# victorvde/jpeg2png

Hardware: NVIDIA H100
Metric: Mpixel-iterations/s (higher is better)
Workload: dtype f32

## Files before the change

jpeg2png_b200/csrc/kernels_project.cu:

```cuda
#include <cuda_runtime.h>
#include <stdint.h>
#include <stdlib.h>

#include "kernels.cuh"
#include "project_generic_body.cuh"
#include "numerics.cuh"
#include "project_common.cuh"
#include "strip_sync.cuh"
#include "tma_maps.h"


namespace j2p {

cudaError_t launch_project_tile(const FrameDev &F, int c, int count, float factor, cudaStream_t s, int *nlaunch, bool uncovered_only);
cudaError_t configure_project_tma();
bool project_tma_enabled();
cudaError_t launch_project_tma(const FrameDev &F, const TileMaps &M, int c, int count, int xsel, float factor, cudaStream_t s);
cudaError_t configure_project_tile22();
cudaError_t launch_project_tile22(const FrameDev &F, int c, int count, float factor, cudaStream_t s, int *nlaunch, bool uncovered_only);

template <int SW, int SH>
__global__ void __launch_bounds__(P_NT, (SW * SH <= 1) ? J2P_PROJ_MIN_CTAS : 2) k_project(const __grid_constant__ FrameDev F, const ProjPlane G, const float factor) {
    constexpr bool REC = false;
    const RecDev R{};
#include "project_generic_body.inc"
}

struct QTable { float q[64]; };
__global__ void __launch_bounds__(P_NT) k_decode(const int16_t *data, const __grid_constant__ QTable qt, float *out, int cw, int ch) {
    const float *q = qt.q;
    __shared__ __align__(16) float tiles[P_NT / 8][TILE_STRIDE];
    const int tid = threadIdx.x, b = tid >> 3, j = tid & 7;
    const int nb = (cw >> 3) * (ch >> 3);
    const int blk = blockIdx.x * (P_NT / 8) + b;
    if (blk >= nb) return;
    const int bw = cw >> 3, by = blk / bw, bx = blk - by * bw;
    float v[8];
// ... 24 lines not shown

cudaError_t configure_project_kernels() {
    const char *e = getenv("J2P_PROJ_TILE22");
    g_tile22 = !(e && *e == '0');
    const cudaError_t rc = configure_project_tma();
    return rc != cudaSuccess ? rc : configure_project_tile22();
}

__global__ void k_fold_sums(const double *sums_by_rank, int nranks, int nc, float *norms) {
    const int c = threadIdx.x;
    if (c >= nc) return;
    double s = 0.;
    for (int r = 0; r < nranks; r++) s = __dadd_rn(s, sums_by_rank[r * 3 + c]);
    const float norm = fsqrt(__double2float_rn(s));
    norms[c] = norm;
    norms[4 + c] = __frcp_rn(norm);
}

cudaError_t launch_fold_sums(const double *sums_by_rank, int nranks, int nc, float *norms, cudaStream_t s) {
    k_fold_sums<<<1, 32, 0, s>>>(sums_by_rank, nranks, nc, norms);
    return cudaGetLastError();
}

cudaError_t launch_project(const FrameDev &Fin, float factor, cudaStream_t s, int *nlaunch) {
    *nlaunch = 0;
    FrameDev F = Fin;
    if (F.t0 != 0 || F.t1 != F.H) {
        const size_t off = (size_t)F.t0 * F.W;
        for (int c = 0; c < F.nc; c++) {
            F.pl[c].x += off;
            F.pl[c].xp += off;
            F.pl[c].g += off;
        }
        F.H = F.t1 - F.t0;
    }
    for (int c = 0; c < F.nc; c++) {
        const PlaneDev &P = F.pl[c];
        const int tw = 8 * P_BW * P.sw, th = 8 * P_BH * P.sh;
        ProjPlane G;
        G.c = c;
        G.gx = (F.W + tw - 1) / tw;
        const int gy = (F.H + th - 1) / th;
        auto each_rows = [&](const FrameDev &V, auto launch) {
            for (int y0 = 0; y0 < gy; y0 += kMaxGridRows) {
                const int rows = gy - y0 < kMaxGridRows ? gy - y0 : kMaxGridRows;
                launch(y0 == 0 && rows == gy ? V : rows_view(V, c, 1, y0 * P_BH, 8 * P.sh, y0 + rows == gy), dim3(G.gx, rows));
                *nlaunch += 1;
            }
        };
        if (F.log_on && P.sw == 1 && P.sh == 1) {
            each_rows(F, [&](const FrameDev &V, dim3 grid) { k_project<1, 1><<<grid, P_NT, 0, s>>>(V, G, factor); });
        } else if (P.sw == 1 && P.sh == 1) {
            int count = 1;
            while (c + count < F.nc && F.pl[c + count].sw == 1 && F.pl[c + count].sh == 1 && F.pl[c + count].cw == P.cw &&
                   F.pl[c + count].ch == P.ch)
                count++;
            const bool tma = Fin.host_maps != nullptr && project_tma_enabled();
            if (tma) {
                const cudaError_t et = launch_project_tma(Fin, *static_cast<const TileMaps *>(Fin.host_maps), c, count, Fin.buf_sel, factor, s);
                if (et != cudaSuccess) return et;
                *nlaunch += 1;
            }
            const cudaError_t eb = launch_project_tile(F, c, count, factor, s, nlaunch, tma);
            if (eb != cudaSuccess) return eb;
            c += count - 1;
        }
        else if (P.sw == 2 && P.sh == 2 && g_tile22 && !F.log_on) {
            int count = 1;
            while (c + count < F.nc && F.pl[c + count].sw == 2 && F.pl[c + count].sh == 2 && F.pl[c + count].cw == P.cw &&
                   F.pl[c + count].ch == P.ch)
                count++;
            const cudaError_t eb = launch_project_tile22(F, c, count, factor, s, nlaunch, false);
            if (eb != cudaSuccess) return eb;
            c += count - 1;
        }
        else {
            for (int f = 0; f < F.nframes; f++) {
                each_rows(F.nframes > 1 ? frame_view(F, f) : F, [&](const FrameDev &V, dim3 grid) {
                    if (P.sw == 2 && P.sh == 2) k_project<2, 2><<<grid, P_NT, 0, s>>>(V, G, factor);
                    else if (P.sw == 2 && P.sh == 1) k_project<2, 1><<<grid, P_NT, 0, s>>>(V, G, factor);
                    else if (P.sw == 1 && P.sh == 2) k_project<1, 2><<<grid, P_NT, 0, s>>>(V, G, factor);
                    else k_project<0, 0><<<grid, P_NT, 0, s>>>(V, G, factor);
                });
            }
        }
        const cudaError_t e = cudaGetLastError();
// ... 24 lines not shown
```

jpeg2png_b200/csrc/kernels_project_tile.cu:

```cuda
#include <cuda_runtime.h>
#include <stdint.h>

#include "project_tile_body.cuh"

namespace j2p {

template <bool RES, bool BATCH>
__global__ void __launch_bounds__(PT_NT, J2P_TILE_MIN_CTAS) k_project_tile(const __grid_constant__ FrameDev F, const int c0, const float factor) {
    const GridGeo geo{};
    constexpr bool REC = false;
    const RecDev R{};
#include "project_tile_body.inc"
}

template <bool BATCH>
__global__ void k_step_uncovered(const __grid_constant__ FrameDev F, const int c, const float factor) {
    step_uncovered_body<BATCH>(F, c, factor, GridGeo{});
}

static cudaError_t launch_step_uncovered(const FrameDev &F, int c, float factor, cudaStream_t s) {
    const PlaneDev &P = F.pl[c];
    const size_t n = (size_t)(F.H - P.ch) * F.W + (size_t)P.ch * (F.W - P.cw);
    int blocks = (int)((n + 255) / 256);
    if (F.nframes > 1) {
        const int cap = (132 * 8 + F.nframes - 1) / F.nframes;
        k_step_uncovered<true><<<dim3(blocks < cap ? blocks : cap, 1, F.nframes), 256, 0, s>>>(F, c, factor);
        return cudaGetLastError();
    }
    if (blocks > 132 * 8) blocks = 132 * 8;
    k_step_uncovered<false><<<blocks, 256, 0, s>>>(F, c, factor);
    return cudaGetLastError();
}

int project_tile_border_units(const PlaneDev &P) { return ((P.cw >> 3) + PT_NB - 1) / PT_NB; }

cudaError_t launch_project_tile(const FrameDev &F, int c, int count, float factor, cudaStream_t s, int *nlaunch, bool uncovered_only) {
    const PlaneDev &P = F.pl[c];
    const int bw = P.cw >> 3, bh = P.ch >> 3, gx = (bw + PT_NB - 1) / PT_NB;
    const bool batch = F.nframes > 1;
    cudaError_t e = cudaSuccess;
    for (int y0 = 0; y0 < bh && !uncovered_only && e == cudaSuccess; y0 += kMaxGridRows) {
        const int rows = bh - y0 < kMaxGridRows ? bh - y0 : kMaxGridRows;
        const FrameDev V = y0 == 0 && rows == bh ? F : rows_view(F, c, count, y0, 8, y0 + rows == bh);
        const dim3 grid = batch ? dim3(gx * count, rows, F.nframes) : dim3(gx, rows, count);
        if (batch)
            e = P.resample ? launch_chain(k_project_tile<true, true>, grid, dim3(PT_NT), 0, s, V, c, factor) : launch_chain(k_project_tile<false, true>, grid, dim3(PT_NT), 0, s, V, c, factor);
        else
            e = P.resample ? launch_chain(k_project_tile<true, false>, grid, dim3(PT_NT), 0, s, V, c, factor) : launch_chain(k_project_tile<false, false>, grid, dim3(PT_NT), 0, s, V, c, factor);
        *nlaunch += 1;
    }
    for (int k = c; k < c + count && e == cudaSuccess; k++)
        if (F.pl[k].cw < F.W || F.pl[k].ch < F.H) {
            e = launch_step_uncovered(F, k, factor, s);
            *nlaunch += 1;
        }
    return e;
}

}
```

jpeg2png_b200/csrc/pdl.cuh:

```cuda
#pragma once
#include <cuda_runtime.h>
#include <stdlib.h>

#include <utility>

namespace j2p {

#ifdef __CUDACC__
__device__ __forceinline__ void pdl_wait() { asm volatile("griddepcontrol.wait;" ::: "memory"); }
__device__ __forceinline__ void pdl_launch_dependents() { asm volatile("griddepcontrol.launch_dependents;" ::: "memory"); }
#endif

inline bool pdl_enabled() {
    static const bool on = [] {
        const char *e = getenv("J2P_PDL");
        return !(e && *e == '0');
    }();
    return on;
}

template <typename... KArgs, typename... Args>
inline cudaError_t launch_chain(void (*kernel)(KArgs...), dim3 grid, dim3 block, size_t smem, cudaStream_t s, Args &&...args) {
    cudaLaunchConfig_t cfg = {};
    cfg.gridDim = grid;
    cfg.blockDim = block;
    cfg.dynamicSmemBytes = smem;
    cfg.stream = s;
    cudaLaunchAttribute attr[1];
    attr[0].id = cudaLaunchAttributeProgrammaticStreamSerialization;
    attr[0].val.programmaticStreamSerializationAllowed = pdl_enabled() ? 1 : 0;
    cfg.attrs = attr;
    cfg.numAttrs = 1;
    return cudaLaunchKernelEx(&cfg, kernel, std::forward<Args>(args)...);
}

}
```

jpeg2png_b200/csrc/session.cu:

```cuda
#include <cuda_runtime.h>

#include <math.h>
#include <stdarg.h>
#include <stdio.h>
#include <stdlib.h>
#include <string.h>
#include <sys/mman.h>
#include <time.h>

#include <atomic>
#include <algorithm>
#include <map>
#include <string>
#include <mutex>
#include <utility>
#include <vector>

#include "../../include/jpeg2png_b200.h"
#include "copy_pool.h"
#include "geometry.cuh"
#include "kernels.cuh"
#include "record.cuh"
#include "tma_maps.h"

namespace j2p {
int grad_cta_count(int W, int H);
cudaError_t configure_kernels(int *slots);
cudaError_t launch_gradient(const FrameDev &F, float factor, cudaStream_t s);
cudaError_t launch_project(const FrameDev &F, float factor, cudaStream_t s, int *nlaunch);
cudaError_t launch_fold_sums(const double *sums_by_rank, int nranks, int nc, float *norms, cudaStream_t s);
cudaError_t launch_decode(const int16_t *data, const float *q_host, float *out, int cw, int ch, cudaStream_t s);
cudaError_t launch_init_plane(const float *fdata, float *x, float *xp, int W, int H, int cw, int ch, int sw, int sh,
                              cudaStream_t s);
bool project_tma_enabled();
int project_tma_border_units(const PlaneDev &P);
int project_tile_border_units(const PlaneDev &P);
cudaError_t launch_scanlines(const EpilogueArgs &a, int nframes, cudaStream_t s, int *nlaunch);
cudaError_t launch_halo_exchange(const HaloPeers &P, unsigned seq, unsigned *ticket, int *err, int wait_for_arrival, cudaStream_t s);
int packed_gradient_gpm(const FrameDev &F);
void packed_gradient_geometry(const FrameDev &F, int *cx, int *bands, int *rows);
cudaError_t launch_project_tile(const FrameDev &F, int c, int count, float factor, cudaStream_t s, int *nlaunch, bool uncovered_only);
cudaError_t launch_project_tile22(const FrameDev &F, int c, int count, float factor, cudaStream_t s, int *nlaunch, bool uncovered_only);
}

using namespace j2p;

static thread_local char g_err[512] = "";

static int fail(int code, const char *fmt, ...) {
    va_list ap;
    va_start(ap, fmt);
    vsnprintf(g_err, sizeof g_err, fmt, ap);
    va_end(ap);
    return code;
}

#define CK(call)                                                                                      \
    do {                                                                                              \
        cudaError_t e_ = (call);                                                                      \
        if (e_ != cudaSuccess) {                                                                      \
            cudaGetLastError();    \
            return fail(J2P_ERR_CUDA, "%s failed: %s (%s:%d)", #call, cudaGetErrorString(e_), __FILE__, __LINE__); \
        }                                                                                             \
    } while (0)

constexpr int kEventRing = 32;
constexpr unsigned kEventStride = 4;

// ... 101 lines not shown
    unsigned next_iter = 0;
    unsigned long long launches = 0;
    int logging = 0;
    double log_host[8] = {};
    long long log_host_iter = -1;
    unsigned long long next_log_iter = 0;
    cudaEvent_t ev[kEventRing] = {};
    long long ev_iter[kEventRing];
    std::vector<std::pair<void *, size_t>> dev_blocks;
    void *stage[kStageSlots] = {};
    cudaEvent_t stage_ev[kStageSlots] = {};
    unsigned stage_next = 0;
    cudaEvent_t export_ev = nullptr;
    cudaEvent_t upload_ev = nullptr;
    unsigned long long uid = 0;
    unsigned long long tables_gen = 0;
    struct GroupPlan *group = nullptr;
    cudaEvent_t group_ev = nullptr;
    bool recording = false;
    bool rec_armed = false;
    double *rec_hist = nullptr;
    double *rec_pp = nullptr;
    unsigned rec_pp_stride = 0, rec_pp_count[3] = {};
};
static void free_group_plan(GroupPlan *g);

static void swap_iterates(FrameDev &F) {
    for (int c = 0; c < F.nc; c++) {
        PlaneDev &P = F.pl[c];
        float *tp = P.x; P.x = P.xp; P.xp = tp;
    }
    F.buf_sel ^= 1;
}

template <typename T>
static cudaError_t dev_alloc(j2p_session *s, T **p, size_t bytes) {
    bytes = bytes ? (bytes + 255) & ~(size_t)255 : 256;
    size_t got = bytes;
    void *q = g_dev_cache.get(s->device, bytes, &got);
    if (!q) {
        got = bytes;
        cudaError_t e = cudaMalloc(&q, bytes);
        if (e == cudaErrorMemoryAllocation) {
            cudaGetLastError();
            g_dev_cache.trim(s->device);
            e = cudaMalloc(&q, bytes);
// ... 51 lines not shown
    if (s && !x) fail(J2P_ERR_ARG, "plane %u out of range (%zu planes)", plane, s->uploaded.size());
    return x;
}
extern "C" unsigned long long j2p_session_launches(const j2p_session *s) { return s ? s->launches : 0; }

extern "C" void j2p_session_destroy(j2p_session *s) {
    if (!s) return;
    cudaSetDevice(s->device);
    if (s->stream) cudaStreamSynchronize(s->stream);
    for (auto &blk : s->dev_blocks)
        if (s->ipc_exported || !g_dev_cache.put(s->device, blk.first, blk.second)) cudaFree(blk.first);
    for (int i = 0; i < kEventRing; i++)
        if (s->ev[i]) cudaEventDestroy(s->ev[i]);
    for (int k = 0; k < kStageSlots; k++) {
        if (s->stage_ev[k]) cudaEventDestroy(s->stage_ev[k]);
        if (s->stage[k]) g_pinned.put(s->stage[k]);
    }
    if (s->export_ev) cudaEventDestroy(s->export_ev);
    if (s->upload_ev) cudaEventDestroy(s->upload_ev);
    if (s->group_ev) cudaEventDestroy(s->group_ev);
    free_group_plan(s->group);
    if (s->stream) cudaStreamDestroy(s->stream);
    delete s;
}

static int create_impl(j2p_session *s, int device, const j2p_frame_desc *d, unsigned row0, unsigned rows, unsigned nframes) {
    const int ndev = j2p_device_count();
    if (ndev <= 0) return fail(J2P_ERR_NODEVICE, "no CUDA device available (the solver has no CPU fallback)");
    if (device < 0 || device >= ndev) return fail(J2P_ERR_ARG, "device %d out of range (0..%d)", device, ndev - 1);
    if (d->nchannel < 1 || d->nchannel > 3) return fail(J2P_ERR_ARG, "nchannel must be 1..3 (compute.c:118)");
    s->device = device;
    s->desc = *d;
    CK(cudaSetDevice(device));
    if (device >= 64) return fail(J2P_ERR_ARG, "device ordinal %d not supported", device);
    std::call_once(g_cfg_once[device], [&] {
        int major = 0, minor = 0;
        cudaError_t e = cudaDeviceGetAttribute(&major, cudaDevAttrComputeCapabilityMajor, device);
        if (e == cudaSuccess) e = cudaDeviceGetAttribute(&minor, cudaDevAttrComputeCapabilityMinor, device);
        g_cfg_cc[device] = major * 10 + minor;
        g_cfg_err[device] = e != cudaSuccess ? e : (major * 10 + minor == 90 ? configure_kernels(&g_cfg_slots[device]) : cudaSuccess);
    });
    if (g_cfg_cc[device] != 90)
        return fail(J2P_ERR_NODEVICE, "device %d is sm_%d; this library is built for sm_90a only", device, g_cfg_cc[device]);
    CK(g_cfg_err[device]);

    FrameDev &F = s->F;
// ... 106 lines not shown
    for (unsigned c = 0; c < d->nchannel && maps_ok; c++) {
        const bool p11 = d->w_samp[c] == 1 && d->h_samp[c] == 1, p22 = d->w_samp[c] == 2 && d->h_samp[c] == 2;
        if (!p11 && !p22) continue;
        const int box_rows = p11 ? 8 : 16;
        maps_ok = encode_plane_map(&s->maps.m[c][0], s->x[c], F.W, F.H, box_rows) == 0 &&
                  encode_plane_map(&s->maps.m[c][1], s->xp[c], F.W, F.H, box_rows) == 0 &&
                  encode_plane_map(&s->maps.m[c][2], s->g[c], F.W, F.H, box_rows) == 0;
        if (maps_ok && p11) maps_ok = encode_plane_map(&s->maps.m[c][3], s->gp[c], F.pl[c].cw, F.pl[c].ch, 8) == 0;
    }
    F.host_maps = maps_ok ? &s->maps : nullptr;
    F.buf_sel = 0;
    F.grad_ctas = grad_cta_count(F.W, F.t1 - F.t0);
    F.grad_slots = g_cfg_slots[device];
    CK(dev_alloc(s, &F.partials, sizeof(double) * 5 * (size_t)F.grad_ctas * nframes));
    CK(dev_alloc(s, &F.norms, sizeof(float) * 16 * nframes));
    CK(dev_alloc(s, &F.sums, sizeof(double) * 4 * nframes));
    CK(dev_alloc(s, &F.logsums, sizeof(double) * 8));
    CK(cudaMemsetAsync(F.logsums, 0, sizeof(double) * 8, s->stream));
    F.log_on = 0;
    F.log_slot = 0;
    CK(dev_alloc(s, &F.counter, sizeof(unsigned) * nframes));
    CK(cudaMemsetAsync(F.counter, 0, sizeof(unsigned) * nframes, s->stream));
    CK(cudaMemsetAsync(F.norms, 0, sizeof(float) * 16 * nframes, s->stream));
    return J2P_OK;
}

extern "C" int j2p_session_create(j2p_session **out, int device, const struct j2p_frame_desc *d) {
    return j2p_session_create_strip(out, device, d, 0, 0);
}

static int create_session(j2p_session **out, int device, const struct j2p_frame_desc *d, unsigned row0, unsigned rows,
                          unsigned nframes) {
    if (!out || !d) return fail(J2P_ERR_ARG, "null argument");
    *out = nullptr;
    j2p_session *s = new j2p_session();
    static std::atomic<unsigned long long> uid_seq{0};
    s->uid = ++uid_seq;
    const int rc = create_impl(s, device, d, row0, rows, nframes);
    if (rc != J2P_OK) {
        char keep[sizeof g_err];
        memcpy(keep, g_err, sizeof keep);
        j2p_session_destroy(s);
        cudaGetLastError();
        memcpy(g_err, keep, sizeof keep);
        return rc;
    }
// ... 8 lines not shown

extern "C" int j2p_session_create_batch(j2p_session **out, int device, const struct j2p_frame_desc *d, unsigned nframes) {
    if (out) *out = nullptr;
    if (nframes == 0) return fail(J2P_ERR_ARG, "a batch needs at least one frame");
    if (nframes > 65535) return fail(J2P_ERR_ARG, "a batch holds at most 65535 frames (%u requested)", nframes);
    return create_session(out, device, d, 0, 0, nframes);
}

extern "C" unsigned j2p_session_frames(const j2p_session *s) { return s ? s->nframes : 0; }

static int refuse_batch(const j2p_session *s, const char *what) {
    return fail(J2P_ERR_ARG, "%s is not available on a batch session (%u frames)", what, s->nframes);
}

static int reset_impl(j2p_session *s) {
    FrameDev &F = s->F;
    for (size_t k = 0; k < s->uploaded.size(); k++)
        if (!s->uploaded[k]) return fail(J2P_ERR_ARG, "plane %zu (frame %zu, channel %zu) has not been uploaded", k, k / F.nc, k % F.nc);
    F.buf_sel = 0;
    for (int c = 0; c < F.nc; c++) {
        PlaneDev &P = F.pl[c];
        P.x = s->x[c];
        P.xp = s->xp[c];
    }
    for (unsigned f = 0; f < s->nframes; f++) {
        const size_t fo = (size_t)f * F.frame_stride;
        for (int c = 0; c < F.nc; c++) {
            PlaneDev &P = F.pl[c];
            const size_t off = (size_t)F.t0 * F.W;
            CK(launch_init_plane(s->fdata0[c] + f * s->fdata_stride, P.x + fo + off, P.xp + fo + off, F.W, F.t1 - F.t0, P.cw, P.ch, P.sw,
                                 P.sh, s->stream));
            s->launches++;
            CK(cudaMemsetAsync(P.gp + fo, 0, (size_t)P.cw * P.ch * sizeof(float), s->stream));
        }
    }
    if (s->dev_tables && s->tables_stale) {
        CK(cudaMemcpyAsync(s->dev_tables, s->tables.data(), s->tables.size() * sizeof(float), cudaMemcpyHostToDevice, s->stream));
        s->tables_stale = false;
    }
    s->stale = false;
    s->t = 1.f;
    s->next_iter = 0;
    for (int i = 0; i < kEventRing; i++) s->ev_iter[i] = -1;
    s->next_log_iter = 0;
    s->log_host_iter = -1;
    CK(cudaMemsetAsync(F.logsums, 0, sizeof(double) * 8, s->stream));
// ... 304 lines not shown
    if (!s) return fail(J2P_ERR_ARG, "null session");
    if (s->nframes > 1) return refuse_batch(s, "j2p_session_copy_halo_to_prev");
    CK(cudaSetDevice(s->device));
    const FrameDev &F = s->F;
    const size_t W = (size_t)F.W;
    for (int c = 0; c < F.nc; c++) {
        if (F.t0 > 0) CK(cudaMemcpyAsync(F.pl[c].xp, F.pl[c].x, (size_t)F.t0 * W * sizeof(float), cudaMemcpyDeviceToDevice, s->stream));
        if (F.t1 < F.H)
            CK(cudaMemcpyAsync(F.pl[c].xp + (size_t)F.t1 * W, F.pl[c].x + (size_t)F.t1 * W, (size_t)(F.H - F.t1) * W * sizeof(float),
                               cudaMemcpyDeviceToDevice, s->stream));
    }
    return J2P_OK;
}

extern "C" int j2p_session_strip_info(const j2p_session *s, unsigned *local_rows, unsigned *first_owned, unsigned *owned_rows) {
    if (!s) return fail(J2P_ERR_ARG, "null session");
    if (s->nframes > 1) return refuse_batch(s, "j2p_session_strip_info");
    if (local_rows) *local_rows = (unsigned)s->F.H;
    if (first_owned) *first_owned = (unsigned)s->F.t0;
    if (owned_rows) *owned_rows = (unsigned)(s->F.t1 - s->F.t0);
    return J2P_OK;
}

extern "C" int j2p_session_iterate(j2p_session *s, unsigned first, unsigned n) {
    if (!s) return fail(J2P_ERR_ARG, "null session");
    if (s->strip) return fail(J2P_ERR_ARG, "a strip session is driven with j2p_session_gradient / j2p_session_project");
    CK(cudaSetDevice(s->device));
    if (s->recording) {
        if ((unsigned long long)first + n > s->desc.iterations)
            return fail(J2P_ERR_ARG, "the objective record holds %u iterations; iterations %u..%llu asked for", s->desc.iterations, first,
                        (unsigned long long)first + n - 1);
        if (first != 0 && !s->rec_armed && !s->stale)
            return fail(J2P_ERR_ARG, "recording was switched on after iteration 0: iterate from first == 0 to re-arm the record");
    }
    int rc = check_ready(s, first);
    if (rc != J2P_OK) return rc;
    for (unsigned i = first; i < first + n; i++) {
        rc = one_iteration(s, i, nullptr, nullptr, nullptr);
        if (rc != J2P_OK) return rc;
        if (i % kEventStride == kEventStride - 1) {
            const int slot = (int)((i / kEventStride) % kEventRing);
            CK(cudaEventRecord(s->ev[slot], s->stream));
            s->ev_iter[slot] = (long long)i;
        }
    }
    s->next_iter = first + n;
    return J2P_OK;
}

extern "C" int j2p_session_profile(j2p_session *s, unsigned n, float *ms_gradient, float *ms_project) {
    if (!s || !ms_gradient || !ms_project || n == 0) return fail(J2P_ERR_ARG, "bad argument");
    CK(cudaSetDevice(s->device));
    if (s->recording && n > s->desc.iterations)
        return fail(J2P_ERR_ARG, "the objective record holds %u iterations; %u asked for", s->desc.iterations, n);
    int rc = check_ready(s, 0);
    if (rc != J2P_OK) return rc;
    cudaEvent_t e[3];
    for (int k = 0; k < 3; k++) CK(cudaEventCreate(&e[k]));
    double sg = 0., sp = 0.;
    for (unsigned i = 0; i < n; i++) {
        rc = one_iteration(s, i, e[0], e[1], e[2]);
        if (rc != J2P_OK) return rc;
        CK(cudaEventSynchronize(e[2]));
        float a = 0.f, b = 0.f;
        CK(cudaEventElapsedTime(&a, e[0], e[1]));
        CK(cudaEventElapsedTime(&b, e[1], e[2]));
// ... 345 lines not shown
    const FrameDev V = record_view(s);
    const RecDev R = record_args(s, iter);
    int cx, bands, rows;
    packed_gradient_geometry(V, &cx, &bands, &rows);
    CK((cudaError_t)objective_api().gradient(&V, factor, cx, bands, rows, packed_gradient_gpm(V), &R, (void *)s->stream));
    return J2P_OK;
}

static int record_project(j2p_session *s, unsigned iter, float factor, int *nlaunch) {
    const FrameDev V = record_view(s);
    const RecDev R = record_args(s, iter);
    *nlaunch = 0;
    for (int c = 0; c < V.nc; c++) {
        const PlaneDev &P = V.pl[c];
        const bool p11 = P.sw == 1 && P.sh == 1, p22 = P.sw == 2 && P.sh == 2;
        int count = 1;
        while ((p11 || p22) && c + count < V.nc && V.pl[c + count].sw == P.sw && V.pl[c + count].sh == P.sh && V.pl[c + count].cw == P.cw &&
               V.pl[c + count].ch == P.ch)
            count++;
        int n = 0;
        CK((cudaError_t)objective_api().project(&V, c, count, factor, &R, (void *)s->stream, &n));
        *nlaunch += n;
        n = 0;
        if (p11) CK(launch_project_tile(s->F, c, count, factor, s->stream, &n, true));
        else if (p22) CK(launch_project_tile22(s->F, c, count, factor, s->stream, &n, true));
        *nlaunch += n;
        c += count - 1;
    }
    return J2P_OK;
}

extern "C" int j2p_session_record_objective(j2p_session *s, int enabled) {
    if (!s) return fail(J2P_ERR_ARG, "null session");
    if (!enabled) {
        s->recording = false;
        s->rec_armed = false;
        return J2P_OK;
    }
    if (s->strip) return fail(J2P_ERR_ARG, "the objective cannot be recorded on a strip session");
    if (s->logging) return fail(J2P_ERR_ARG, "the session logs the objective (j2p_session_set_logging); recording is the other way to get it");
    const ObjectiveApi &api = objective_api();
    if (!api.gradient) return fail(J2P_ERR_CUDA, "%s", api.err);
    CK(cudaSetDevice(s->device));
    std::call_once(g_objective_once[s->device & 63], [&] { g_objective_cfg[s->device & 63] = api.configure(); });
    CK((cudaError_t)g_objective_cfg[s->device & 63]);
    if (!s->rec_hist) {
        unsigned stride = 1;
// ... 671 lines not shown
```

Before: 24110.

## Fuse projection and gradient into one per-iteration kernel with ping-pong buffers

Adds a fused step kernel that does the DCT-domain projection for a band of block rows and then computes the TV/TGV gradient from a shared-memory window, so each iteration needs one launch instead of separate project and gradient launches. New x and gradient buffers are allocated and rotated each iteration so the fused kernel writes outputs without clobbering neighbouring bands' inputs. The aim is to cut global-memory round trips and launch overhead between the two stages. The cost is extra memory, recomputation of halo rows, and higher register and shared-memory pressure. The fused path is used only for single-frame, non-strip sessions with enough band rows and no TMA, logging or recording; it also makes PDL chaining of the final project launch optional.

```diff
diff --git a/jpeg2png_b200/csrc/kernels_project.cu b/jpeg2png_b200/csrc/kernels_project.cu
--- a/jpeg2png_b200/csrc/kernels_project.cu
+++ b/jpeg2png_b200/csrc/kernels_project.cu
@@ -12,7 +12,7 @@
 
 namespace j2p {
 
-cudaError_t launch_project_tile(const FrameDev &F, int c, int count, float factor, cudaStream_t s, int *nlaunch, bool uncovered_only);
+cudaError_t launch_project_tile(const FrameDev &F, int c, int count, float factor, cudaStream_t s, int *nlaunch, bool uncovered_only, bool chained);
 cudaError_t configure_project_tma();
 bool project_tma_enabled();
 cudaError_t launch_project_tma(const FrameDev &F, const TileMaps &M, int c, int count, int xsel, float factor, cudaStream_t s);
@@ -83,7 +83,7 @@
     return cudaGetLastError();
 }
 
-cudaError_t launch_project(const FrameDev &Fin, float factor, cudaStream_t s, int *nlaunch) {
+cudaError_t launch_project(const FrameDev &Fin, float factor, cudaStream_t s, int *nlaunch, bool chained) {
     *nlaunch = 0;
     FrameDev F = Fin;
     if (F.t0 != 0 || F.t1 != F.H) {
@@ -122,7 +122,7 @@
                 if (et != cudaSuccess) return et;
                 *nlaunch += 1;
             }
-            const cudaError_t eb = launch_project_tile(F, c, count, factor, s, nlaunch, tma);
+            const cudaError_t eb = launch_project_tile(F, c, count, factor, s, nlaunch, tma, chained);
             if (eb != cudaSuccess) return eb;
             c += count - 1;
         }
diff --git a/jpeg2png_b200/csrc/kernels_project_tile.cu b/jpeg2png_b200/csrc/kernels_project_tile.cu
--- a/jpeg2png_b200/csrc/kernels_project_tile.cu
+++ b/jpeg2png_b200/csrc/kernels_project_tile.cu
@@ -34,7 +34,7 @@
 
 int project_tile_border_units(const PlaneDev &P) { return ((P.cw >> 3) + PT_NB - 1) / PT_NB; }
 
-cudaError_t launch_project_tile(const FrameDev &F, int c, int count, float factor, cudaStream_t s, int *nlaunch, bool uncovered_only) {
+cudaError_t launch_project_tile(const FrameDev &F, int c, int count, float factor, cudaStream_t s, int *nlaunch, bool uncovered_only, bool chained) {
     const PlaneDev &P = F.pl[c];
     const int bw = P.cw >> 3, bh = P.ch >> 3, gx = (bw + PT_NB - 1) / PT_NB;
     const bool batch = F.nframes > 1;
@@ -46,7 +46,8 @@
         if (batch)
             e = P.resample ? launch_chain(k_project_tile<true, true>, grid, dim3(PT_NT), 0, s, V, c, factor) : launch_chain(k_project_tile<false, true>, grid, dim3(PT_NT), 0, s, V, c, factor);
         else
-            e = P.resample ? launch_chain(k_project_tile<true, false>, grid, dim3(PT_NT), 0, s, V, c, factor) : launch_chain(k_project_tile<false, false>, grid, dim3(PT_NT), 0, s, V, c, factor);
+            e = P.resample ? launch_chain_if(chained, k_project_tile<true, false>, grid, dim3(PT_NT), 0, s, V, c, factor)
+                           : launch_chain_if(chained, k_project_tile<false, false>, grid, dim3(PT_NT), 0, s, V, c, factor);
         *nlaunch += 1;
     }
     for (int k = c; k < c + count && e == cudaSuccess; k++)
diff --git a/jpeg2png_b200/csrc/kernels_step_fused.cu b/jpeg2png_b200/csrc/kernels_step_fused.cu
--- /dev/null
+++ b/jpeg2png_b200/csrc/kernels_step_fused.cu
@@ -0,0 +1,515 @@
+#include <cuda_runtime.h>
+#include <stdint.h>
+
+#include "gradient_common.cuh"
+#include "gradient_packed_body.cuh"
+#include "kernels.cuh"
+#include "numerics.cuh"
+#include "pdl.cuh"
+#include "project_common.cuh"
+#include "project_tile_body.cuh"
+
+namespace j2p {
+
+constexpr int FS_NT = GM_NT;
+constexpr int FS_BLK = GM_WARPS * GM_USE / 8 + 2;
+constexpr int FS_ROWS = 11;
+constexpr int FS_LD = 8 * FS_BLK + 4;
+constexpr int FS_HALF = PT_NB;
+static_assert(FS_BLK == 2 * FS_HALF, "two blocks per thread cover the window");
+template <int NC>
+struct FusedSmem {
+    float win[2][NC][FS_ROWS][FS_LD];
+    float4 stage[3][8][2 * PT_C4];
+    int4 data[2][FS_NT];
+};
+
+__device__ __forceinline__ void fdct8x8_rows_x2(float (&a)[8], float (&b)[8], float *tile_a, float *tile_b, int j) {
+    const int h = (j >> 2) & 1;
+    {
+        float4 *ra = reinterpret_cast<float4 *>(tile_a + j * 8), *rb = reinterpret_cast<float4 *>(tile_b + j * 8);
+        ra[h] = make_float4(a[0], a[1], a[2], a[3]);
+        ra[h ^ 1] = make_float4(a[4], a[5], a[6], a[7]);
+        rb[h] = make_float4(b[0], b[1], b[2], b[3]);
+        rb[h ^ 1] = make_float4(b[4], b[5], b[6], b[7]);
+    }
+    __syncwarp();
+#pragma unroll
+    for (int i = 0; i < 8; i++) {
+        const int o = i * 8 + (j ^ (((i >> 2) & 1) << 2));
+        a[i] = tile_a[o];
+        b[i] = tile_b[o];
+    }
+    __syncwarp();
+    fdct8(a);
+    fdct8(b);
+#pragma unroll
+    for (int i = 0; i < 8; i++) {
+        const int o = i * 8 + (j ^ (((i >> 2) & 1) << 2));
+        tile_a[o] = a[i];
+        tile_b[o] = b[i];
+    }
+    __syncwarp();
+    {
+        const float4 *ra = reinterpret_cast<const float4 *>(tile_a + j * 8), *rb = reinterpret_cast<const float4 *>(tile_b + j * 8);
+        const float4 al = ra[h], ah = ra[h ^ 1], bl = rb[h], bh = rb[h ^ 1];
+        a[0] = al.x; a[1] = al.y; a[2] = al.z; a[3] = al.w; a[4] = ah.x; a[5] = ah.y; a[6] = ah.z; a[7] = ah.w;
+        b[0] = bl.x; b[1] = bl.y; b[2] = bl.z; b[3] = bl.w; b[4] = bh.x; b[5] = bh.y; b[6] = bh.z; b[7] = bh.w;
+    }
+    __syncwarp();
+    fdct8(a);
+    fdct8(b);
+}
+
+template <int NC, bool TGV>
+__global__ void __launch_bounds__(FS_NT, 2) k_step_fused(const __grid_constant__ FrameDev F, float *const x_out, float *const g_out,
+                                                        const float fproj, const float factor, const int band_rows) {
+    extern __shared__ __align__(16) unsigned char fs_raw[];
+    FusedSmem<NC> &S = *reinterpret_cast<FusedSmem<NC> *>(fs_raw);
+    __shared__ __align__(16) float tiles[2][PT_NT / 8][TILE_STRIDE];
+    __shared__ __align__(16) float sq[NC][3][64];
+    __shared__ float snorm[NC][2];
+
+    const int tid = threadIdx.x, lane = tid & 31, wid = tid >> 5;
+    const int W = F.W, H = F.H, bw = W >> 3;
+    const unsigned PS = F.plane_stride;
+    const int yb = blockIdx.y * band_rows;
+    const int ye = min(yb + band_rows, H);
+    const int cb0 = (int)blockIdx.x * (FS_BLK - 2) - 1;
+    const int R0 = max(yb - 2, 0) >> 3, R1 = min(ye + 2, H - 1) >> 3;
+
+    pdl_wait();
+    pdl_launch_dependents();
+
+    for (int e = tid; e < NC * 64; e += FS_NT) {
+        const int c = e >> 6, k = e & 63;
+        sq[c][0][k] = F.q[c][k];
+        sq[c][1][k] = F.qq[c][k];
+        sq[c][2][k] = F.rqq[c][k];
+    }
+    if (tid < NC) {
+        snorm[tid][0] = F.norms[tid];
+        snorm[tid][1] = F.norms[4 + tid];
+    }
+
+    const int nrounds = (R1 - R0 + 1) * NC;
+    auto issue = [&](int q) {
+        const int R = R0 + q / NC, c = q % NC;
+        const PlaneDev &P = F.pl[c];
+#pragma unroll
+        for (int i = 0; i < 4; i++) {
+            const int e = tid + FS_NT * i, row = e >> (PT_SH + 1), c4 = e & (2 * PT_C4 - 1), blk = cb0 + (c4 >> 1);
+            if (blk >= 0 && blk < bw) {
+                const size_t gi = (size_t)(8 * R + row) * W + (size_t)blk * 8 + (c4 & 1) * 4;
+                cp_async16(&S.stage[0][row][c4 ^ row], P.x + gi);
+                cp_async16(&S.stage[1][row][c4 ^ row], P.xp + gi);
+                cp_async16(&S.stage[2][row][c4 ^ row], P.g + gi);
+            }
+        }
+#pragma unroll
+        for (int u = 0; u < 2; u++) {
+            const int blk = cb0 + u * FS_HALF + (tid >> 3);
+            if (blk >= 0 && blk < bw) cp_async16(&S.data[u][tid], P.data + ((size_t)(R * bw + blk) * 64 + (tid & 7) * 8));
+        }
+        cp_async_commit();
+    };
+
+    const f2 fac = splat(factor), one = splat(F.one);
+    auto project = [&](int q) {
+        const int R = R0 + q / NC, c = q % NC;
+        const PlaneDev &P = F.pl[c];
+        const int b = tid >> 3, j = tid & 7;
+        Stepper stepper;
+        stepper.factor = fproj;
+        stepper.step = F.step;
+        stepper.norm = snorm[c][0];
+        stepper.rn = snorm[c][1];
+        stepper.stepping = stepper.norm != 0.f;
+        const bool norm_ok = qdiv_divisor_ok(stepper.norm);
+        const bool use_prob = P.use_prob != 0;
+
+        float v[2][8], xk[2][8];
+        int4 draw[2];
+#pragma unroll
+        for (int u = 0; u < 2; u++) {
+            const int wb = u * FS_HALF + b;
+            unsigned key = 0xffffffffu;
+#pragma unroll
+            for (int hh = 0; hh < 2; hh++) {
+                const int pc = (2 * wb + hh) ^ j;
+                const float4 a = S.stage[0][j][pc], p = S.stage[1][j][pc], g = S.stage[2][j][pc];
+                v[u][hh * 4 + 0] = stepper.fast(a.x, p.x, g.x, key);
+                v[u][hh * 4 + 1] = stepper.fast(a.y, p.y, g.y, key);
+                v[u][hh * 4 + 2] = stepper.fast(a.z, p.z, g.z, key);
+                v[u][hh * 4 + 3] = stepper.fast(a.w, p.w, g.w, key);
+                xk[u][hh * 4 + 0] = a.x; xk[u][hh * 4 + 1] = a.y; xk[u][hh * 4 + 2] = a.z; xk[u][hh * 4 + 3] = a.w;
+            }
+            if (stepper.stepping && !(norm_ok && key >= QDIV_KEY_MIN)) {
+#pragma unroll
+                for (int hh = 0; hh < 2; hh++) {
+                    const int pc = (2 * wb + hh) ^ j;
+                    const float4 a = S.stage[0][j][pc], p = S.stage[1][j][pc], g = S.stage[2][j][pc];
+                    v[u][hh * 4 + 0] = stepper(a.x, p.x, g.x);
+                    v[u][hh * 4 + 1] = stepper(a.y, p.y, g.y);
+                    v[u][hh * 4 + 2] = stepper(a.z, p.z, g.z);
+                    v[u][hh * 4 + 3] = stepper(a.w, p.w, g.w);
+                }
+            }
+            draw[u] = S.data[u][tid];
+        }
+        __syncthreads();
+        if (q + 1 < nrounds) issue(q + 1);
+
+        fdct8x8_rows_x2(v[0], v[1], tiles[0][b], tiles[1][b], j);
+
+        float r[2][8];
+        {
+            const float4 *t0 = reinterpret_cast<const float4 *>(&sq[c][0][j * 8]);
+            const float4 *t1 = reinterpret_cast<const float4 *>(&sq[c][1][j * 8]);
+            const float4 *t2 = reinterpret_cast<const float4 *>(&sq[c][2][j * 8]);
+            float qv[8], qqv[8], rqv[8];
+#pragma unroll
+            for (int k = 0; k < 2; k++) {
+                const float4 a = t0[k], bq = t1[k], cq = t2[k];
+                qv[k * 4] = a.x; qv[k * 4 + 1] = a.y; qv[k * 4 + 2] = a.z; qv[k * 4 + 3] = a.w;
+                qqv[k * 4] = bq.x; qqv[k * 4 + 1] = bq.y; qqv[k * 4 + 2] = bq.z; qqv[k * 4 + 3] = bq.w;
+                rqv[k * 4] = cq.x; rqv[k * 4 + 1] = cq.y; rqv[k * 4 + 2] = cq.z; rqv[k * 4 + 3] = cq.w;
+            }
+#pragma unroll
+            for (int u = 0; u < 2; u++) {
+                const int dw[4] = {draw[u].x, draw[u].y, draw[u].z, draw[u].w};
+                float num[8];
+                unsigned rkey = 0xffffffffu;
+#pragma unroll
+                for (int i = 0; i < 8; i++) {
+                    const int di = (i & 1) ? (dw[i >> 1] >> 16) : (int)(short)(dw[i >> 1] & 0xffff);
+                    const float d = (float)di;
+                    const float qf = qv[i];
+                    const float lo_ = fmul(fsub(d, 0.5f), qf), hi_ = fmul(fadd(d, 0.5f), qf);
+                    float t = v[u][i];
+                    t = t > hi_ ? hi_ : (t < lo_ ? lo_ : t);
+                    v[u][i] = t;
+                    num[i] = fsub(t, fmul(d, qf));
+                    rkey = min(rkey, qdiv_key(num[i]));
+                    r[u][i] = qdiv_core(num[i], qqv[i], rqv[i]);
+                }
+                if (rkey < QDIV_KEY_MIN) {
+#pragma unroll
+                    for (int i = 0; i < 8; i++) r[u][i] = fdiv(num[i], qqv[i]);
+                }
+            }
+        }
+
+        idct8x8_rows_x2(v[0], v[1], tiles[0][b], tiles[1][b], j);
+        if (use_prob) idct8x8_rows_x2(r[0], r[1], tiles[0][b], tiles[1][b], j);
+
+        const float pa = P.p_alpha;
+        const bool row_owned = 8 * R >= yb && 8 * R < ye;
+        float *xo = x_out + (size_t)c * PS + (size_t)(8 * R + j) * W;
+#pragma unroll
+        for (int u = 0; u < 2; u++) {
+            const int wb = u * FS_HALF + b, blk = cb0 + wb;
+            float *wy = &S.win[0][c][3 + j][wb * 8];
+            float *wg = &S.win[1][c][3 + j][wb * 8];
+#pragma unroll
+            for (int hh = 0; hh < 2; hh++) {
+                const f2 x0 = pk(v[u][hh * 4 + 0], v[u][hh * 4 + 1]), x1 = pk(v[u][hh * 4 + 2], v[u][hh * 4 + 3]);
+                const f2 y0 = addm2(mul2(fac, sub2(x0, pk(xk[u][hh * 4 + 0], xk[u][hh * 4 + 1]))), x0, one);
+                const f2 y1 = addm2(mul2(fac, sub2(x1, pk(xk[u][hh * 4 + 2], xk[u][hh * 4 + 3]))), x1, one);
+                reinterpret_cast<float4 *>(wy)[hh] = make_float4(lo(y0), hi(y0), lo(y1), hi(y1));
+                reinterpret_cast<float4 *>(wg)[hh] = use_prob ? make_float4(fmul(pa, r[u][hh * 4 + 0]), fmul(pa, r[u][hh * 4 + 1]),
+                                                                            fmul(pa, r[u][hh * 4 + 2]), fmul(pa, r[u][hh * 4 + 3]))
+                                                              : make_float4(0.f, 0.f, 0.f, 0.f);
+            }
+            if (row_owned && wb >= 1 && wb <= FS_BLK - 2 && blk < bw) {
+                float4 *dst = reinterpret_cast<float4 *>(xo + (size_t)blk * 8);
+                dst[0] = make_float4(v[u][0], v[u][1], v[u][2], v[u][3]);
+                dst[1] = make_float4(v[u][4], v[u][5], v[u][6], v[u][7]);
+            }
+        }
+    };
+
+    const int X0 = ((int)blockIdx.x * GM_WARPS + wid) * GM_USE;
+    const int px0 = X0 - 2 + 2 * lane;
+    const bool pair_in = px0 >= 0 && px0 < W;
+    const bool is_target = pair_in && lane >= 1 && lane <= 30;
+    const bool has_l0 = px0 > 0, has_r1 = px0 + 1 < W - 1;
+    const f2 a1s = splat(F.a1), a1n = splat(-F.a1), a2s = splat(F.a2), a2n = splat(-F.a2), a2m2 = splat(fmul(-2.f, F.a2));
+    const f2 half2 = splat(0.5f), zero2 = 0ull;
+    const unsigned zero = (unsigned)band_rows >> 31;
+    const int pxw = (pair_in ? px0 : (px0 < 0 ? 0 : W - 2)) - 8 * cb0;
+
+    double acc[NC];
+    RowCarry<NC> A, B;
+    f2 gmask[NC];
+#pragma unroll
+    for (int c = 0; c < NC; c++) {
+        acc[c] = 0.;
+        A.y[c] = A.gx[c] = A.gy[c] = A.og[c] = A.tvb[c] = A.ud[c] = A.dg[c] = zero2;
+        gmask[c] = splat(F.pl[c].use_prob ? 1.f : 0.f);
+    }
+    A.ok1 = A.ok2 = true;
+
+    int Rcur = R0;
+    auto row_step = [&](const int i, const RowCarry<NC> &P, RowCarry<NC> &N) {
+        const int wr = min(max(i, 0), H - 1) - 8 * Rcur + 3;
+        const int wg = min(max(i - 1, yb), ye - 1) - 8 * Rcur + 3;
+        unsigned ykey = 0xffffffffu;
+        f2 pterm[NC];
+#pragma unroll
+        for (int c = 0; c < NC; c++) {
+            const float2 vy = *reinterpret_cast<const float2 *>(&S.win[0][c][wr][pxw]);
+            N.y[c] = pk(vy.x, vy.y);
+            ykey = min(ykey, min(qdiv_key(lo(N.y[c])), qdiv_key(hi(N.y[c]))));
+            const float2 vg = *reinterpret_cast<const float2 *>(&S.win[1][c][wg][pxw]);
+            pterm[c] = fma2(pk(vg.x, vg.y), gmask[c], zero2);
+        }
+
+        const int s = i - 1;
+        const bool src_in = pair_in & (s >= 0) & (s < H);
+
+        f2 gx0[NC], gy0[NC];
+        f2 n1 = zero2;
+#pragma unroll
+        for (int c = 0; c < NC; c++) {
+            float yr1 = __shfl_down_sync(0xffffffffu, lo(P.y[c]), 1);
+            yr1 = has_r1 ? yr1 : hi(P.y[c]);
+            gx0[c] = sub2(shr_from_right(P.y[c], yr1), P.y[c]);
+            gy0[c] = sub2(N.y[c], P.y[c]);
+            const f2 sx = mul2(gx0[c], gx0[c]), sy = mul2(gy0[c], gy0[c]);
+            n1 = c == 0 ? addm2(sy, sx, one) : addm2(sy, addm2(sx, n1, one), one);
+            N.gx[c] = gx0[c];
+            N.gy[c] = gy0[c];
+        }
+        const bool tl0 = src_in & (lo(n1) != 0.f), tl1 = src_in & (hi(n1) != 0.f);
+        const f2 ss1 = pk(tl0 ? lo(n1) : 1.f, tl1 ? hi(n1) : 1.f);
+        bool bad = (ykey < QDIV_YKEY_MIN) | !root_arg_ok(lo(ss1)) | !root_arg_ok(hi(ss1));
+
+        f2 gxx[NC], gyy[NC], sym[NC];
+        f2 ss2 = zero2;
+        bool gl0 = false, gl1 = false;
+        if (TGV) {
+            f2 gyPv[NC];
+#pragma unroll
+            for (int c = 0; c < NC; c++) gyPv[c] = P.gy[c];
+            if (__builtin_expect(s <= 0, false)) {
+#pragma unroll
+                for (int c = 0; c < NC; c++) gyPv[c] = gy0[c];
+            }
+            f2 n2 = zero2;
+#pragma unroll
+            for (int c = 0; c < NC; c++) {
+                float gxl = __shfl_up_sync(0xffffffffu, hi(gx0[c]), 1);
+                float gyl = __shfl_up_sync(0xffffffffu, hi(gy0[c]), 1);
+                gxl = has_l0 ? gxl : lo(gx0[c]);
+                gyl = has_l0 ? gyl : lo(gy0[c]);
+                gxx[c] = sub2(gx0[c], shl_from_left(gx0[c], gxl));
+                const f2 gyx = sub2(gy0[c], shl_from_left(gy0[c], gyl));
+                const f2 gxy = sub2(gx0[c], P.gx[c]);
+                gyy[c] = sub2(gy0[c], gyPv[c]);
+                const f2 u = add2(gxy, gyx);
+                sym[c] = mul2(u, half2);
+                const f2 t = addm2(mul2(gyy[c], gyy[c]), addm2(mul2(u, sym[c]), mul2(gxx[c], gxx[c]), one), one);
+                n2 = c == 0 ? t : add2(n2, t);
+            }
+            gl0 = src_in & (lo(n2) != 0.f);
+            gl1 = src_in & (hi(n2) != 0.f);
+            ss2 = pk(gl0 ? lo(n2) : 1.f, gl1 ? hi(n2) : 1.f);
+            bad = bad | !root_arg_ok(lo(ss2)) | !root_arg_ok(hi(ss2));
+        }
+
+        const bool ok0 = !__any_sync(0xffffffffu, bad);
+        N.ok1 = ok0;
+        N.ok2 = P.ok1;
+        const bool fast = ok0 && P.ok1 && P.ok2;
+
+        f2 tvs0[NC], tvr0[NC], t2s0[NC], lr0[NC];
+        {
+            const f2 n = sqrt2_core(ss1), nb = neg2(n);
+            const f2 yr = rcp2_core(n, nb);
+            const f2 y = pk(tl0 ? lo(yr) : 0.f, tl1 ? hi(yr) : 0.f);
+            const f2 yl = rcp2_low(nb, y);
+#pragma unroll
+            for (int c = 0; c < NC; c++) {
+                tvs0[c] = qdiv2x(mul2(a1n, add2(gx0[c], gy0[c])), nb, y, yl);
+                tvr0[c] = qdiv2x(mul2(a1s, gx0[c]), nb, y, yl);
+                N.tvb[c] = qdiv2x(mul2(a1s, gy0[c]), nb, y, yl);
+            }
+        }
+        if (TGV) {
+            const f2 n = sqrt2_core(ss2), nb = neg2(n);
+            const f2 yr = rcp2_core(n, nb);
+            const f2 y = pk(gl0 ? lo(yr) : 0.f, gl1 ? hi(yr) : 0.f);
+            const f2 yl = rcp2_low(nb, y);
+#pragma unroll
+            for (int c = 0; c < NC; c++) {
+                const f2 sx = addm2(sym[c], gxx[c], one);
+                t2s0[c] = mul2(a2m2, qdiv2x(add2(sx, gyy[c]), nb, y, yl));
+                lr0[c] = mul2(a2s, qdiv2x(sx, nb, y, yl));
+                N.ud[c] = mul2(a2s, qdiv2x(addm2(sym[c], gyy[c], one), nb, y, yl));
+                N.dg[c] = mul2(a2n, qdiv2x(sym[c], nb, y, yl));
+            }
+        } else {
+#pragma unroll
+            for (int c = 0; c < NC; c++) t2s0[c] = lr0[c] = N.ud[c] = N.dg[c] = zero2;
+        }
+        if (__builtin_expect(!fast, false)) {
+            {
+                TvSlow<NC> io;
+#pragma unroll
+                for (int c = 0; c < NC; c++) {
+                    io.gx[c][0] = lo(gx0[c]); io.gx[c][1] = hi(gx0[c]);
+                    io.gy[c][0] = lo(gy0[c]); io.gy[c][1] = hi(gy0[c]);
+                }
+                tv_slow<NC>(&io, F.a1, src_in);
+#pragma unroll
+                for (int c = 0; c < NC; c++) {
+                    tvs0[c] = pk(settle(io.q[0][c][0], zero), settle(io.q[0][c][1], zero));
+                    tvr0[c] = pk(settle(io.q[1][c][0], zero), settle(io.q[1][c][1], zero));
+                    N.tvb[c] = pk(settle(io.q[2][c][0], zero), settle(io.q[2][c][1], zero));
+                }
+            }
+            if (TGV) {
+                TgvSlow<NC> io;
+#pragma unroll
+                for (int c = 0; c < NC; c++) {
+                    io.gxx[c][0] = lo(gxx[c]); io.gxx[c][1] = hi(gxx[c]);
+                    io.gyy[c][0] = lo(gyy[c]); io.gyy[c][1] = hi(gyy[c]);
+                    io.sym[c][0] = lo(sym[c]); io.sym[c][1] = hi(sym[c]);
+                }
+                tgv_slow<NC>(&io, F.a2, src_in);
+#pragma unroll
+                for (int c = 0; c < NC; c++) {
+                    t2s0[c] = pk(settle(io.q[0][c][0], zero), settle(io.q[0][c][1], zero));
+                    lr0[c] = pk(settle(io.q[1][c][0], zero), settle(io.q[1][c][1], zero));
+                    N.ud[c] = pk(settle(io.q[2][c][0], zero), settle(io.q[2][c][1], zero));
+                    N.dg[c] = pk(settle(io.q[3][c][0], zero), settle(io.q[3][c][1], zero));
+                }
+            }
+        }
+
+        {
+            const bool st = is_target & (i >= yb + 2) & (i <= ye + 1);
+            const unsigned ro = (unsigned)max(s - 1, 0) * (unsigned)W;
+#pragma unroll
+            for (int c = 0; c < NC; c++) {
+                f2 o = P.og[c];
+                if (TGV) {
+                    const float dgl = __shfl_up_sync(0xffffffffu, hi(N.dg[c]), 1);
+                    o = addm2(N.ud[c], add2(o, shl_from_left(N.dg[c], dgl)), one);
+                }
+                if (st) *reinterpret_cast<float2 *>(g_out + (ro + c * PS + (unsigned)px0)) = make_float2(lo(o), hi(o));
+                const f2 sq2 = mul2(o, o);
+                acc[c] = __dadd_rn(acc[c], (double)(st ? lo(sq2) : 0.f));
+                acc[c] = __dadd_rn(acc[c], (double)(st ? hi(sq2) : 0.f));
+            }
+        }
+
+#pragma unroll
+        for (int c = 0; c < NC; c++) {
+            const float tvr_l = __shfl_up_sync(0xffffffffu, hi(tvr0[c]), 1);
+            f2 o = add2(add2(add2(pterm[c], P.tvb[c]), shl_from_left(tvr0[c], tvr_l)), tvs0[c]);
+            if (TGV) {
+                const float dg_r = __shfl_down_sync(0xffffffffu, lo(P.dg[c]), 1);
+                o = add2(addm2(P.ud[c], o, one), shr_from_right(P.dg[c], dg_r));
+                const float lr_l = __shfl_up_sync(0xffffffffu, hi(lr0[c]), 1);
+                const float lr_r = __shfl_down_sync(0xffffffffu, lo(lr0[c]), 1);
+                o = add2(addm2(t2s0[c], add2(o, shl_from_left(lr0[c], lr_l)), one), shr_from_right(lr0[c], lr_r));
+            }
+            N.og[c] = o;
+        }
+    };
+
+    issue(0);
+    int i = yb - 2;
+    for (int q = 0; q < nrounds; q++) {
+        cp_async_wait<0>();
+        __syncthreads();
+        project(q);
+        if ((q + 1) % NC == 0) {
+            __syncthreads();
+            const int avail = min(8 * Rcur + 7, H - 1);
+            while (i <= ye + 1 && max(min(i + 1, H - 1), min(max(i, yb), ye - 1)) <= avail) {
+                row_step(i, A, B);
+                row_step(i + 1, B, A);
+                i += 2;
+            }
+            __syncthreads();
+            for (int e = tid; e < 2 * NC * 3 * (FS_LD / 4); e += FS_NT) {
+                const int a = e / (NC * 3 * (FS_LD / 4)), rest = e % (NC * 3 * (FS_LD / 4));
+                const int c = rest / (3 * (FS_LD / 4)), rr = (rest / (FS_LD / 4)) % 3, c4 = rest % (FS_LD / 4);
+                reinterpret_cast<float4 *>(S.win[a][c][rr])[c4] = reinterpret_cast<const float4 *>(S.win[a][c][8 + rr])[c4];
+            }
+            Rcur++;
+        }
+    }
+
+    __shared__ double red[3][GM_WARPS];
+    __shared__ unsigned ticket;
+#pragma unroll
+    for (int c = 0; c < NC; c++) {
+        const double sum = warp_sum(acc[c]);
+        if (lane == 0) red[c][wid] = sum;
+    }
+    __syncthreads();
+    const unsigned cta = blockIdx.y * gridDim.x + blockIdx.x, ncta = gridDim.x * gridDim.y;
+    if (tid == 0) {
+#pragma unroll
+        for (int c = 0; c < NC; c++) {
+            double sum = 0.;
+            for (int k = 0; k < GM_WARPS; k++) sum = __dadd_rn(sum, red[c][k]);
+            F.partials[(size_t)c * F.grad_ctas + cta] = sum;
+        }
+        unsigned t;
+        asm volatile("atom.release.gpu.global.add.u32 %0, [%1], 1;" : "=r"(t) : "l"(F.counter) : "memory");
+        ticket = t;
+    }
+    __syncthreads();
+    if (ticket == ncta - 1) {
+        __threadfence();
+#pragma unroll
+        for (int c = 0; c < NC; c++) {
+            double sum = 0.;
+            for (unsigned k = tid; k < ncta; k += FS_NT) sum = __dadd_rn(sum, __ldcg(&F.partials[(size_t)c * F.grad_ctas + k]));
+            sum = warp_sum(sum);
+            if (lane == 0) red[c][wid] = sum;
+        }
+        __syncthreads();
+        if (tid < NC) {
+            double sum = 0.;
+            for (int k = 0; k < GM_WARPS; k++) sum = __dadd_rn(sum, red[tid][k]);
+            const float norm = fsqrt(__double2float_rn(sum));
+            F.sums[tid] = sum;
+            F.norms[tid] = norm;
+            F.norms[4 + tid] = __frcp_rn(norm);
+        }
+        if (tid == 0) *F.counter = 0u;
+    }
+}
+
+template <int NC, bool TGV>
+static cudaError_t launch_nc(const FrameDev &F, float *x_out, float *g_out, float fproj, float factor, int cx, int bands, int rows,
+                             cudaStream_t s) {
+    static const cudaError_t cfg = cudaFuncSetAttribute(k_step_fused<NC, TGV>, cudaFuncAttributeMaxDynamicSharedMemorySize,
+                                                        (int)sizeof(FusedSmem<NC>));
+    if (cfg != cudaSuccess) return cfg;
+    return launch_chain(k_step_fused<NC, TGV>, dim3(cx, bands), dim3(FS_NT), sizeof(FusedSmem<NC>), s, F, x_out, g_out, fproj, factor, rows);
+}
+
+}
+
+using namespace j2p;
+
+extern "C" int j2p_fused_step(const FrameDev *F, float *x_out, float *g_out, float fproj, float factor, int cx, int bands, int rows,
+                              cudaStream_t s) {
+    cudaError_t e;
+    switch (F->nc) {
+        case 1: e = F->use_tgv ? launch_nc<1, true>(*F, x_out, g_out, fproj, factor, cx, bands, rows, s)
+                               : launch_nc<1, false>(*F, x_out, g_out, fproj, factor, cx, bands, rows, s); break;
+        case 2: e = F->use_tgv ? launch_nc<2, true>(*F, x_out, g_out, fproj, factor, cx, bands, rows, s)
+                               : launch_nc<2, false>(*F, x_out, g_out, fproj, factor, cx, bands, rows, s); break;
+        default: e = F->use_tgv ? launch_nc<3, true>(*F, x_out, g_out, fproj, factor, cx, bands, rows, s)
+                                : launch_nc<3, false>(*F, x_out, g_out, fproj, factor, cx, bands, rows, s); break;
+    }
+    return (int)e;
+}
diff --git a/jpeg2png_b200/csrc/pdl.cuh b/jpeg2png_b200/csrc/pdl.cuh
--- a/jpeg2png_b200/csrc/pdl.cuh
+++ b/jpeg2png_b200/csrc/pdl.cuh
@@ -20,7 +20,7 @@
 }
 
 template <typename... KArgs, typename... Args>
-inline cudaError_t launch_chain(void (*kernel)(KArgs...), dim3 grid, dim3 block, size_t smem, cudaStream_t s, Args &&...args) {
+inline cudaError_t launch_chain_if(bool chained, void (*kernel)(KArgs...), dim3 grid, dim3 block, size_t smem, cudaStream_t s, Args &&...args) {
     cudaLaunchConfig_t cfg = {};
     cfg.gridDim = grid;
     cfg.blockDim = block;
@@ -28,10 +28,14 @@
     cfg.stream = s;
     cudaLaunchAttribute attr[1];
     attr[0].id = cudaLaunchAttributeProgrammaticStreamSerialization;
-    attr[0].val.programmaticStreamSerializationAllowed = pdl_enabled() ? 1 : 0;
+    attr[0].val.programmaticStreamSerializationAllowed = chained && pdl_enabled() ? 1 : 0;
     cfg.attrs = attr;
     cfg.numAttrs = 1;
     return cudaLaunchKernelEx(&cfg, kernel, std::forward<Args>(args)...);
 }
+template <typename... KArgs, typename... Args>
+inline cudaError_t launch_chain(void (*kernel)(KArgs...), dim3 grid, dim3 block, size_t smem, cudaStream_t s, Args &&...args) {
+    return launch_chain_if(true, kernel, grid, block, smem, s, std::forward<Args>(args)...);
+}
 
 }
diff --git a/jpeg2png_b200/csrc/session.cu b/jpeg2png_b200/csrc/session.cu
--- a/jpeg2png_b200/csrc/session.cu
+++ b/jpeg2png_b200/csrc/session.cu
@@ -27,7 +27,7 @@
 int grad_cta_count(int W, int H);
 cudaError_t configure_kernels(int *slots);
 cudaError_t launch_gradient(const FrameDev &F, float factor, cudaStream_t s);
-cudaError_t launch_project(const FrameDev &F, float factor, cudaStream_t s, int *nlaunch);
+cudaError_t launch_project(const FrameDev &F, float factor, cudaStream_t s, int *nlaunch, bool chained = true);
 cudaError_t launch_fold_sums(const double *sums_by_rank, int nranks, int nc, float *norms, cudaStream_t s);
 cudaError_t launch_decode(const int16_t *data, const float *q_host, float *out, int cw, int ch, cudaStream_t s);
 cudaError_t launch_init_plane(const float *fdata, float *x, float *xp, int W, int H, int cw, int ch, int sw, int sh,
@@ -39,11 +39,15 @@
 cudaError_t launch_halo_exchange(const HaloPeers &P, unsigned seq, unsigned *ticket, int *err, int wait_for_arrival, cudaStream_t s);
 int packed_gradient_gpm(const FrameDev &F);
 void packed_gradient_geometry(const FrameDev &F, int *cx, int *bands, int *rows);
-cudaError_t launch_project_tile(const FrameDev &F, int c, int count, float factor, cudaStream_t s, int *nlaunch, bool uncovered_only);
+cudaError_t launch_project_tile(const FrameDev &F, int c, int count, float factor, cudaStream_t s, int *nlaunch, bool uncovered_only,
+                                bool chained);
 cudaError_t launch_project_tile22(const FrameDev &F, int c, int count, float factor, cudaStream_t s, int *nlaunch, bool uncovered_only);
 }
 
 using namespace j2p;
+
+extern "C" int j2p_fused_step(const FrameDev *F, float *x_out, float *g_out, float fproj, float factor, int cx, int bands, int rows,
+                              cudaStream_t s);
 
 static thread_local char g_err[512] = "";
 
@@ -191,6 +195,9 @@
     double *rec_hist = nullptr;
     double *rec_pp = nullptr;
     unsigned rec_pp_stride = 0, rec_pp_count[3] = {};
+    bool fused = false;
+    float *x2[3] = {}, *g2[3] = {};
+    float *x_free[3] = {}, *g_free[3] = {};
 };
 static void free_group_plan(GroupPlan *g);
 
@@ -288,6 +295,14 @@
     free_group_plan(s->group);
     if (s->stream) cudaStreamDestroy(s->stream);
     delete s;
+}
+
+constexpr int kFusedMinBandRows = 32;
+static bool fused_geometry(const FrameDev &F) {
+    if (packed_gradient_gpm(F) != 1 || F.H / 8 > kMaxGridRows) return false;
+    int cx, bands, rows;
+    packed_gradient_geometry(F, &cx, &bands, &rows);
+    return rows >= kFusedMinBandRows;
 }
 
 static int create_impl(j2p_session *s, int device, const j2p_frame_desc *d, unsigned row0, unsigned rows, unsigned nframes) {
@@ -440,6 +455,17 @@
     CK(dev_alloc(s, &F.counter, sizeof(unsigned) * nframes));
     CK(cudaMemsetAsync(F.counter, 0, sizeof(unsigned) * nframes, s->stream));
     CK(cudaMemsetAsync(F.norms, 0, sizeof(float) * 16 * nframes, s->stream));
+    s->fused = nframes == 1 && !s->strip && fused_geometry(F);
+    if (s->fused) {
+        float *slab2 = nullptr;
+        CK(dev_alloc(s, &slab2, PS * 2 * d->nchannel * sizeof(float)));
+        for (unsigned c = 0; c < d->nchannel; c++) {
+            s->x2[c] = slab2 + PS * c;
+            s->g2[c] = slab2 + PS * (d->nchannel + c);
+            s->x_free[c] = s->x2[c];
+            s->g_free[c] = s->g2[c];
+        }
+    }
     return J2P_OK;
 }
 
@@ -494,6 +520,11 @@
         PlaneDev &P = F.pl[c];
         P.x = s->x[c];
         P.xp = s->xp[c];
+        if (s->fused) {
+            P.g = s->g[c];
+            s->x_free[c] = s->x2[c];
+            s->g_free[c] = s->g2[c];
+        }
     }
     for (unsigned f = 0; f < s->nframes; f++) {
         const size_t fo = (size_t)f * F.frame_stride;
@@ -844,6 +875,52 @@
     return J2P_OK;
 }
 
+static int mark_iteration(j2p_session *s, unsigned i) {
+    if (i % kEventStride == kEventStride - 1) {
+        const int slot = (int)((i / kEventStride) % kEventRing);
+        CK(cudaEventRecord(s->ev[slot], s->stream));
+        s->ev_iter[slot] = (long long)i;
+    }
+    return J2P_OK;
+}
+
+static int iterate_fused(j2p_session *s, unsigned first, unsigned n) {
+    FrameDev &F = s->F;
+    int cx, bands, rows;
+    packed_gradient_geometry(F, &cx, &bands, &rows);
+    auto next_factor = [s] {
+        const float tnext = (1 + sqrtf(1 + 4 * (s->t * s->t))) / 2;
+        const float factor = (s->t - 1) / tnext;
+        s->t = tnext;
+        return factor;
+    };
+    float factor = next_factor();
+    CK(launch_gradient(F, factor, s->stream));
+    s->launches++;
+    for (unsigned i = first; i + 1 < first + n; i++) {
+        const float fnext = next_factor();
+        CK((cudaError_t)j2p_fused_step(&F, s->x_free[0], s->g_free[0], factor, fnext, cx, bands, rows, s->stream));
+        s->launches++;
+        for (int c = 0; c < F.nc; c++) {
+            PlaneDev &P = F.pl[c];
+            float *const xm = P.xp, *const gk = P.g;
+            P.xp = P.x;
+            P.x = s->x_free[c];
+            P.g = s->g_free[c];
+            s->x_free[c] = xm;
+            s->g_free[c] = gk;
+        }
+        const int rc = mark_iteration(s, i);
+        if (rc != J2P_OK) return rc;
+        factor = fnext;
+    }
+    int nproj = 0;
+    CK(launch_project(F, factor, s->stream, &nproj, false));
+    s->launches += (unsigned)nproj;
+    swap_iterates(F);
+    return mark_iteration(s, first + n - 1);
+}
+
 extern "C" int j2p_session_iterate(j2p_session *s, unsigned first, unsigned n) {
     if (!s) return fail(J2P_ERR_ARG, "null session");
     if (s->strip) return fail(J2P_ERR_ARG, "a strip session is driven with j2p_session_gradient / j2p_session_project");
@@ -857,13 +934,15 @@
     }
     int rc = check_ready(s, first);
     if (rc != J2P_OK) return rc;
-    for (unsigned i = first; i < first + n; i++) {
-        rc = one_iteration(s, i, nullptr, nullptr, nullptr);
+    if (s->fused && n >= 2 && !s->recording && !s->F.log_on && !project_tma_enabled()) {
+        rc = iterate_fused(s, first, n);
         if (rc != J2P_OK) return rc;
-        if (i % kEventStride == kEventStride - 1) {
-            const int slot = (int)((i / kEventStride) % kEventRing);
-            CK(cudaEventRecord(s->ev[slot], s->stream));
-            s->ev_iter[slot] = (long long)i;
+    } else {
+        for (unsigned i = first; i < first + n; i++) {
+            rc = one_iteration(s, i, nullptr, nullptr, nullptr);
+            if (rc != J2P_OK) return rc;
+            rc = mark_iteration(s, i);
+            if (rc != J2P_OK) return rc;
         }
     }
     s->next_iter = first + n;
@@ -1255,7 +1334,7 @@
         CK((cudaError_t)objective_api().project(&V, c, count, factor, &R, (void *)s->stream, &n));
         *nlaunch += n;
         n = 0;
-        if (p11) CK(launch_project_tile(s->F, c, count, factor, s->stream, &n, true));
+        if (p11) CK(launch_project_tile(s->F, c, count, factor, s->stream, &n, true, true));
         else if (p22) CK(launch_project_tile22(s->F, c, count, factor, s->stream, &n, true));
         *nlaunch += n;
         c += count - 1;
```

Result: slower. 20420, median of 6 (-15.3%).
